# PFLeget/treegp

Measured on AMD Instinct MI355X. Metric: GP solve+predict throughput, 2-D AnisotropicRBF N=65536, higher is better.
Workload: dtype f64

## Files before the change

### treegp_amd/csrc/chol.hip

```cpp
#include "tgp_internal.h"

#include "gemm_tile.h"
#include "potrf128.h"

#ifdef TGP_POTRF_STAMPS
__device__ unsigned long long tgp_gemm_stamps[1024 * 4];
__device__ int tgp_gemm_stamp_grid = 43;
__device__ unsigned long long tgp_queue_stamps[1024 * 4];
__device__ int tgp_queue_stamp_T = 40;
__device__ unsigned long long tgp_mid_stamps[25 * 8];
__device__ int tgp_mid_stamp_base = 5120;
#define TGP_MID_STAMP(i)                                                                                   \
    do {                                                                                                   \
        if (threadIdx.x == 0 && base == tgp_mid_stamp_base && blockIdx.x < 25) tgp_mid_stamps[blockIdx.x * 8 + (i)] = __builtin_amdgcn_s_memrealtime(); \
    } while (0)
#else
#define TGP_MID_STAMP(i) ((void)0)
#endif

namespace {
template <int MODE, int LDB>
__global__ __launch_bounds__(256, 2) void gemm_col_kernel(const double *A, const double *B, double *C) {
    const int64_t t = blockIdx.x;
    TGP_CHAIN_PRIO();
#ifdef TGP_POTRF_STAMPS
    const unsigned long long t_in = __builtin_amdgcn_s_memrealtime();
#endif
    gemm_tile_128<MODE, LDB, TGP_TB>(A + t * 128 * TGP_PW, B, C + t * 128 * TGP_PW);
#ifdef TGP_POTRF_STAMPS
    if (MODE == 0 && threadIdx.x == 0 && (int)gridDim.x == tgp_gemm_stamp_grid) {
        tgp_gemm_stamps[blockIdx.x * 4 + 0] = t_in;
        tgp_gemm_stamps[blockIdx.x * 4 + 1] = __builtin_amdgcn_s_memrealtime();
        tgp_gemm_stamps[blockIdx.x * 4 + 2] = (__builtin_amdgcn_s_getreg(20 | (0 << 6) | (3 << 11)) << 8) | __builtin_amdgcn_s_getreg(4 | (8 << 6) | (7 << 11));
    }
#endif
}

template <int MODE, int LDB>
__global__ __launch_bounds__(256) void gemm_col_small_kernel(const double *A, const double *B, double *C) {
    const int64_t o = (int64_t)blockIdx.x * 16 * TGP_PW;
    TGP_CHAIN_PRIO();
    nt_slice_tile<MODE, TGP_TB, 1>(nt_slice_lds_storage(), A + o, TGP_PW, B, LDB, C + o, TGP_PW, nullptr, nullptr);
}
__device__ __forceinline__ void keep_w_share(double *__restrict__ keep, const double *__restrict__ W0) {
    if (!keep) return;
    constexpr int n2 = TGP_TB * TGP_TB;
    const int per = (n2 + (int)gridDim.x - 1) / (int)gridDim.x;
    const int lo = (int)blockIdx.x * per, hi = lo + per < n2 ? lo + per : n2;
    for (int i = lo + (int)threadIdx.x; i < hi; i += 256)
        reinterpret_cast<double2 *>(keep)[i] = reinterpret_cast<const double2 *>(W0)[i];
}
__global__ __launch_bounds__(256, 2) void panel_tall_kernel(double *rows0, const double *W0, const double *L10, const double *W1,
                                                            double *keep) {
    double *rows = rows0 + (int64_t)blockIdx.x * 128 * TGP_PW;
    TGP_CHAIN_PRIO();
    keep_w_share(keep, W0);
    gemm_tile_128<0, TGP_TB, TGP_TB>(rows, W0, rows);
    __syncthreads();
    gemm_tile_128<1, TGP_PW, TGP_TB>(rows, L10, rows + TGP_TB);
    __syncthreads();
    gemm_tile_128<0, TGP_TB, TGP_TB>(rows + TGP_TB, W1, rows + TGP_TB);
}

__global__ __launch_bounds__(256) void panel_tall_small_kernel(double *rows0, const double *W0, const double *L10, const double *W1,
                                                               double *keep) {
    double *rows = rows0 + (int64_t)blockIdx.x * 16 * TGP_PW;
    TGP_CHAIN_PRIO();
    keep_w_share(keep, W0);
    double *lds = nt_slice_lds_storage();
    nt_slice_tile<0, TGP_TB, 1>(lds, rows, TGP_PW, W0, TGP_TB, rows, TGP_PW, nullptr, nullptr);
    asm volatile("s_waitcnt vmcnt(0)" ::: "memory");
    __syncthreads();
    nt_slice_tile<1, TGP_TB, 1>(lds, rows, TGP_PW, L10, TGP_PW, rows + TGP_TB, TGP_PW, nullptr, nullptr);
    asm volatile("s_waitcnt vmcnt(0)" ::: "memory");
    __syncthreads();
    nt_slice_tile<0, TGP_TB, 1>(lds, rows + TGP_TB, TGP_PW, W1, TGP_TB, rows + TGP_TB, TGP_PW, nullptr, nullptr);
}

__global__ __launch_bounds__(256, 2) void diag_mid_kernel(double *R1, const double *W0) {
    TGP_CHAIN_PRIO();
    gemm_tile_128<0, TGP_TB, TGP_TB>(R1, W0, R1);
    __syncthreads();
    gemm_tile_128<1, TGP_PW, TGP_TB>(R1, R1, R1 + TGP_TB);
}

constexpr unsigned long long PANEL_SPIN_TICKS = 5000000ull;
constexpr int PANEL_SYNC_WORDS = 16;
__device__ __forceinline__ void panel_publish(unsigned *counter) {
    asm volatile("s_waitcnt vmcnt(0)" ::: "memory");
    __syncthreads();
    if (threadIdx.x == 0) {
        __builtin_amdgcn_fence(__ATOMIC_RELEASE, "agent");
        __hip_atomic_fetch_add(counter, 1u, __ATOMIC_RELAXED, __HIP_MEMORY_SCOPE_AGENT);
    }
}
__device__ __forceinline__ bool panel_wait(unsigned *sync, int which, unsigned target, int *info) {
    __shared__ int s_ok;
    if (threadIdx.x == 0) {
        int ok = 1;
        const unsigned long long t0 = __builtin_amdgcn_s_memrealtime();
        unsigned it = 0;
        while (__hip_atomic_load(sync + which, __ATOMIC_RELAXED, __HIP_MEMORY_SCOPE_AGENT) < target) {
            __builtin_amdgcn_s_sleep(1);
            if ((++it & 63u) == 0u) {
                const bool late = __builtin_amdgcn_s_memrealtime() - t0 > PANEL_SPIN_TICKS;
                if (late || __hip_atomic_load(sync + 2, __ATOMIC_RELAXED, __HIP_MEMORY_SCOPE_AGENT) != 0u) {
                    __hip_atomic_store(sync + 2, 1u, __ATOMIC_RELAXED, __HIP_MEMORY_SCOPE_AGENT);
                    if (late) __hip_atomic_store(info, -7, __ATOMIC_RELAXED, __HIP_MEMORY_SCOPE_AGENT);
                    ok = 0;
                    break;
                }
            }
        }
        __builtin_amdgcn_fence(__ATOMIC_ACQUIRE, "agent");
        s_ok = ok;
    }
    __syncthreads();
    const bool ok = s_ok != 0;
    __syncthreads();
    return ok;
}
template <bool SMALLROWS>
__global__ __launch_bounds__(256) void panel_mid_kernel(double *Pk, const double *W0, double *W1, int *info, int base, unsigned *sync) {
    __shared__ __attribute__((aligned(16))) double T[potrf_v2::POTRF_LDS_DOUBLES];
    static_assert(potrf_v2::POTRF_LDS_DOUBLES >= 2 * 2 * 128 * TileDefault::LS, "the GEMM tile's staging fits in potrf128's image");
    static_assert(potrf_v2::POTRF_LDS_DOUBLES >= NT_SLICE_LDS_DOUBLES, "... and the latency tile's");
    TGP_CHAIN_PRIO();
    const int b = blockIdx.x;
    double *R1 = Pk + (int64_t)TGP_TB * TGP_PW;
    TGP_MID_STAMP(0);
    if (b < 8) {
        double *rows = R1 + (int64_t)b * 16 * TGP_PW;
        nt_slice_tile<0, TGP_TB, 1>(T, rows, TGP_PW, W0, TGP_TB, rows, TGP_PW, nullptr, nullptr);
        TGP_MID_STAMP(1);
        panel_publish(sync + 0);
        TGP_MID_STAMP(2);
        return;
    }
    if (b < 24) {
        if (!panel_wait(sync, 0, 8u, info)) return;
        TGP_MID_STAMP(1);
        double *rows = R1 + (int64_t)((b - 8) >> 1) * 16 * TGP_PW;
        const int64_t ch = (int64_t)(b & 1) * 64;
        nt_slice_tile<1, TGP_TB, 1, 64>(T, rows, TGP_PW, R1 + ch * TGP_PW, TGP_PW, rows + TGP_TB + ch, TGP_PW, nullptr, nullptr);
        TGP_MID_STAMP(2);
        panel_publish(sync + 1);
        TGP_MID_STAMP(3);
        return;
    }
    if (b == 24) {
        if (!panel_wait(sync, 1, 16u, info)) return;
        TGP_MID_STAMP(1);
        potrf_v2::potrf128_body<true>(T, R1 + TGP_TB, TGP_PW, W1, info, base + TGP_TB);
        TGP_MID_STAMP(2);
        return;
    }
    if constexpr (SMALLROWS) {
        double *rows = Pk + (int64_t)TGP_PW * TGP_PW + (int64_t)(b - 25) * 16 * TGP_PW;
        nt_slice_tile<0, TGP_TB, 1>(T, rows, TGP_PW, W0, TGP_TB, rows, TGP_PW, nullptr, nullptr);
        asm volatile("s_waitcnt vmcnt(0)" ::: "memory");
        __syncthreads();
        if (!panel_wait(sync, 0, 8u, info)) return;
        nt_slice_tile<1, TGP_TB, 1>(T, rows, TGP_PW, R1, TGP_PW, rows + TGP_TB, TGP_PW, nullptr, nullptr);
    } else {
        double *rows = Pk + (int64_t)TGP_PW * TGP_PW + (int64_t)(b - 25) * 128 * TGP_PW;
        gemm_tile_128_at<0, TGP_TB, TGP_TB>(T, rows, W0, rows);
        __syncthreads();
        if (!panel_wait(sync, 0, 8u, info)) return;
        gemm_tile_128_at<1, TGP_PW, TGP_TB>(T, rows, R1, rows + TGP_TB);
    }
}

template <int NSEG>
__global__ __launch_bounds__(256) void syrk_small_kernel(double *Abase, int64_t Np, int ob, int T, const double *P0,
                                                         const double *P1) {
    const int ri = blockIdx.x;
    const int tj = blockIdx.y;
    if (tj > (ri >> 3) || (ri >> 3) >= T) return;
    TGP_CHAIN_PRIO();
    const int64_t pj = ob + (tj >> 1);
    const int64_t I = (int64_t)TGP_PW * ob + 16 * (int64_t)ri;
    double *C = Abase + panel_off(pj, Np) + (I - pj * TGP_PW) * TGP_PW + (tj & 1) * TGP_TB;
    const int64_t oa = (int64_t)ri * 16 * TGP_PW, obb = (int64_t)tj * TGP_TB * TGP_PW;
    nt_slice_tile<1, TGP_PW, NSEG>(nt_slice_lds_storage(), P0 + oa, TGP_PW, P0 + obb, TGP_PW, C, TGP_PW, NSEG > 1 ? P1 + oa : nullptr,
                                   NSEG > 1 ? P1 + obb : nullptr);
}

template <int NSEG>
__global__ __launch_bounds__(256, 2) void syrk_dtv_kernel(double *Abase, int64_t Np, int ob, int T, int strip, const double *P0,
                                                          const double *P1, int diag_full) {
    int ti, tj;
    if (strip == 0) {
        tilemap(blockIdx.x, T, ti, tj);
        if (ti < 0) return;
    } else {
        tj = (int)(blockIdx.x % strip);
        ti = (int)(blockIdx.x / strip);
        if (ti < tj || ti >= T) return;
    }
// ... 304 lines not shown
        if (n >= slots_per_class) break;
        syrk_distn_tile<NSEG>(((int64_t)n << 3) | xcd, Aloc, loff, kpanel, G, g, S, col_lo, ncol, nrows, M);
        __syncthreads();
    }
}

inline void run_potrf128(hipStream_t st, double *A, int lda, double *W, int *info, int base, bool exclusive = false, bool solo = false) {
    constexpr unsigned image = potrf_v2::POTRF_LDS_BYTES, full = 128 * 1024;
    static const bool attr_ok = [] {
        return hipFuncSetAttribute((const void *)potrf_v2::potrf128_kernel<true>, hipFuncAttributeMaxDynamicSharedMemorySize, (int)full) == hipSuccess &&
               hipFuncSetAttribute((const void *)potrf_v2::potrf128_solo_kernel, hipFuncAttributeMaxDynamicSharedMemorySize, (int)full) == hipSuccess;
    }();
    (void)attr_ok;
    if (exclusive || solo) potrf_v2::potrf128_solo_kernel<<<1, 256, exclusive ? full : image, st>>>(A, lda, W, info, base);
    else potrf_v2::potrf128_kernel<true><<<1, 256, image, st>>>(A, lda, W, info, base);
}
}

namespace {
__global__ void set_identity128_kernel(double *__restrict__ W) {
    const int t = blockIdx.x * 256 + threadIdx.x;
    W[t] = (t >> 7) == (t & 127) ? 1.0 : 0.0;
}

void factor_panel(hipStream_t st, double *Pk, int64_t mk, double *W0, int *d_info, int base, bool exclusive = false,
                  int64_t n_data = -1, unsigned *mid_sync = nullptr, int cu_budget = 0) {
    double *W1 = W0 + TGP_TB * TGP_TB;
    double *R1 = Pk + (int64_t)TGP_TB * TGP_PW;
    const int r1 = (int)((mk - TGP_TB) / TGP_TB);
    static const int small_rows = [] { const char *e = getenv("TGP_SMALL_ROWS"); return e ? atoi(e) : 80; }();
    const bool solo = cu_budget >= 256 && mid_sync != nullptr;
    run_potrf128(st, Pk, TGP_PW, W0, d_info, base, exclusive, solo);
    if (n_data >= 0 && (int64_t)base + TGP_TB >= n_data && mk == TGP_PW) {
        gemm_col_small_kernel<0, TGP_TB><<<8, 256, 0, st>>>(R1, W0, R1);
        set_identity128_kernel<<<64, 256, 0, st>>>(W1);
        return;
    }
    const int r2 = (int)((mk - TGP_PW) / TGP_TB);
    if (mid_sync) {
        constexpr unsigned pad = 128 * 1024 - potrf_v2::POTRF_LDS_DOUBLES * 8;
        static const bool pad_ok = [] {
            return hipFuncSetAttribute((const void *)panel_mid_kernel<true>, hipFuncAttributeMaxDynamicSharedMemorySize, (int)pad) == hipSuccess &&
                   hipFuncSetAttribute((const void *)panel_mid_kernel<false>, hipFuncAttributeMaxDynamicSharedMemorySize, (int)pad) == hipSuccess;
        }();
        const unsigned dyn = (exclusive && pad_ok) ? pad : 0u;
        if (17 + 8 * r2 <= cu_budget) panel_mid_kernel<true><<<25 + 8 * r2, 256, dyn, st>>>(Pk, W0, W1, d_info, base, mid_sync);
        else panel_mid_kernel<false><<<25 + r2, 256, dyn, st>>>(Pk, W0, W1, d_info, base, mid_sync);
    } else if (cu_budget > 0) {
        double *R2 = Pk + (int64_t)TGP_PW * TGP_PW;
        const bool small = 17 + 8 * r2 <= cu_budget;
        gemm_col_small_kernel<0, TGP_TB><<<8, 256, 0, st>>>(R1, W0, R1);
        if (r2 > 0) {
            if (small) gemm_col_small_kernel<0, TGP_TB><<<r2 * 8, 256, 0, st>>>(R2, W0, R2);
            else gemm_col_kernel<0, TGP_TB><<<r2, 256, 0, st>>>(R2, W0, R2);
        }
        gemm_col_small_kernel<1, TGP_PW><<<8, 256, 0, st>>>(R1, R1, R1 + TGP_TB);
        if (r2 > 0) {
            if (small) gemm_col_small_kernel<1, TGP_PW><<<r2 * 8, 256, 0, st>>>(R2, R1, R2 + TGP_TB);
            else gemm_col_kernel<1, TGP_PW><<<r2, 256, 0, st>>>(R2, R1, R2 + TGP_TB);
        }
        run_potrf128(st, R1 + TGP_TB, TGP_PW, W1, d_info, base + TGP_TB, exclusive, solo);
    } else {
        if (r1 <= small_rows) {
            gemm_col_small_kernel<0, TGP_TB><<<r1 * 8, 256, 0, st>>>(R1, W0, R1);
            gemm_col_small_kernel<1, TGP_PW><<<r1 * 8, 256, 0, st>>>(R1, R1, R1 + TGP_TB);
        } else {
            gemm_col_kernel<0, TGP_TB><<<r1, 256, 0, st>>>(R1, W0, R1);
            gemm_col_kernel<1, TGP_PW><<<r1, 256, 0, st>>>(R1, R1, R1 + TGP_TB);
        }
        run_potrf128(st, R1 + TGP_TB, TGP_PW, W1, d_info, base + TGP_TB, exclusive, solo);
    }
    if (r2 > 0) {
        double *R2 = Pk + (int64_t)TGP_PW * TGP_PW + TGP_TB;
        if (r2 <= small_rows) gemm_col_small_kernel<0, TGP_TB><<<r2 * 8, 256, 0, st>>>(R2, W1, R2);
        else gemm_col_kernel<0, TGP_TB><<<r2, 256, 0, st>>>(R2, W1, R2);
    }
}

inline int diag_full() {
    static const int v = [] { const char *e = getenv("TGP_DIAG_FULL"); return e ? (atoi(e) != 0 ? 1 : 0) : 0; }();
    return v;
}

inline int small_t() {
    static const int v = [] { const char *e = getenv("TGP_SMALL_T"); return e ? atoi(e) : 8; }();
    return v;
}

template <int NSEG>
void launch_syrk(hipStream_t st, double *d_A, int64_t Np, int ob, int T, int strip, const double *P0, const double *P1) {
    if (T <= 0) return;
    static const int strip_small_t = [] { const char *e = getenv("TGP_STRIP_SMALL_T"); return e ? atoi(e) : 16; }();
    if (T <= small_t() || (strip > 0 && T <= strip_small_t)) {
        const int cols = strip == 0 ? T : (strip < T ? strip : T);
        syrk_small_kernel<NSEG><<<dim3((unsigned)(T * 8), (unsigned)cols), 256, 0, st>>>(d_A, Np, ob, T, P0, P1);
        return;
    }
    static const int strip64_t = [] { const char *e = getenv("TGP_STRIP64_T"); return e ? atoi(e) : 128; }();
    static const int strip32_t = [] { const char *e = getenv("TGP_STRIP32_T"); return e ? atoi(e) : 64; }();
    if (strip > 0 && T <= strip32_t) {
        syrk_strip32_kernel<NSEG><<<(unsigned)((int64_t)4 * T * strip), 256, 0, st>>>(d_A, Np, ob, T, strip, P0, P1);
        return;
    }
    if (strip > 0 && T <= strip64_t) {
        syrk_strip64_kernel<NSEG><<<(unsigned)((int64_t)2 * T * strip), 256, 0, st>>>(d_A, Np, ob, T, strip, P0, P1);
        return;
    }
    const unsigned gs = strip == 0 ? (unsigned)tilemap_grid(T) : (unsigned)((int64_t)T * strip);
// ... 228 lines not shown
    }
    TGP_HIP(hipGetLastError());
    TGP_HIP(hipMemcpyAsync(ctx->h_info, ctx->d_info, sizeof(int), hipMemcpyDeviceToHost, st));
    ctx->timings[6] = nlaunch;
    ctx->timings[7] = flops;
    ctx->timings[5] = 0.0;
    if (defer_info && !prof) return 0;
    TGP_HIP(hipStreamSynchronize(st));
    if (prof) {
        double tot = 0.0;
        for (int i = 0; i < nlaunch; ++i) {
            float ms = 0.f;
            TGP_HIP(hipEventElapsedTime(&ms, ctx->prof_events[2 * i], ctx->prof_events[2 * i + 1]));
            tot += ms;
        }
        ctx->timings[5] = tot;
    }
    return tgp_potrf_info_rc(ctx, *ctx->h_info);
}

int tgp_potrf_info_rc(tgp_ctx *ctx, int info) {
    if (info >= 0) return info;
    ctx->err = "Cholesky: an in-kernel hand-off timed out (panel_mid_kernel waited 50 ms for workgroups of its own launch); "
               "the factor is incomplete -- TGP_PANEL_MID=0 selects the schedule without in-kernel waits";
    return TGP_RC_HANDOFF;
}

int launch_factor_diag256(tgp_ctx *ctx, double *blk, double *W0, double *W1, int base, bool latency) {
    hipStream_t st = ctx->stream;
    double *R1 = blk + (int64_t)TGP_TB * TGP_PW;
    const bool excl = ctx->chain_exclusive != 0;
    run_potrf128(st, blk, TGP_PW, W0, ctx->d_info, base, excl);
    if (latency) {
        gemm_col_small_kernel<0, TGP_TB><<<8, 256, 0, st>>>(R1, W0, R1);
        gemm_col_small_kernel<1, TGP_PW><<<8, 256, 0, st>>>(R1, R1, R1 + TGP_TB);
    } else {
        diag_mid_kernel<<<1, 256, 0, st>>>(R1, W0);
    }
    run_potrf128(st, R1 + TGP_TB, TGP_PW, W1, ctx->d_info, base + TGP_TB, excl);
    TGP_HIP(hipGetLastError());
    return 0;
}

int launch_trsm_rows(tgp_ctx *ctx, double *rows, int ntiles, const double *Lkk, const double *W0, const double *W1, double *keepW) {
    if (ntiles <= 0) {
        if (keepW) TGP_HIP(hipMemcpyAsync(keepW, W0, (size_t)2 * TGP_TB * TGP_TB * 8, hipMemcpyDeviceToDevice, ctx->stream));
        return 0;
    }
    constexpr int small_max = 24;
    if (ntiles <= small_max)
        panel_tall_small_kernel<<<ntiles * 8, 256, 0, ctx->stream>>>(rows, W0, Lkk + (int64_t)TGP_TB * TGP_PW, W1, keepW);
    else
        panel_tall_kernel<<<ntiles, 256, 0, ctx->stream>>>(rows, W0, Lkk + (int64_t)TGP_TB * TGP_PW, W1, keepW);
    TGP_HIP(hipGetLastError());
    return 0;
}

template <int NSEG>
static void launch_distn(hipStream_t st, unsigned grid, double *d_Aloc, const int64_t *d_loff, int kpanel, int G, int g,
                         const double *const *P, const int *cmax, int col_lo, int ncol, int nrows, const DistMap &M, int nres,
                         unsigned *queue, const double *const *PB) {
    DistSegs<NSEG> S;
    for (int s = 0; s < NSEG; ++s) {
        S.P[s] = P[s];
        S.PB[s] = PB ? PB[s] : P[s];
        S.cmax[s] = cmax[s];
        S.frg[s] = (int)dist_first_round(kpanel + s + 1, g, G);
// ... 158 lines not shown
```

### treegp_amd/csrc/gemm_tile.h

```cpp
#pragma once
#include "tgp_internal.h"

typedef double d4 __attribute__((ext_vector_type(4)));

constexpr int KB = 16;

template <int LSV, bool PRE>
struct TileCfg {
    static constexpr int LS = LSV;
    static constexpr bool PRELOAD = PRE;
};
using TileDefault = TileCfg<17, true>;

using v2u = __attribute__((ext_vector_type(2))) unsigned;
using v4u = __attribute__((ext_vector_type(4))) unsigned;
__device__ __forceinline__ __amdgpu_buffer_rsrc_t tile_rsrc(const double *p, int bytes) {
    return __builtin_amdgcn_make_buffer_rsrc(const_cast<double *>(p), 0, bytes, 0x00020000);
}
__device__ __forceinline__ double buf_ld1(__amdgpu_buffer_rsrc_t r, int voff, int soff) {
    return __builtin_bit_cast(double, __builtin_amdgcn_raw_buffer_load_b64(r, voff, soff, 0));
}
__device__ __forceinline__ double2 buf_ld2(__amdgpu_buffer_rsrc_t r, int voff, int soff) {
    return __builtin_bit_cast(double2, __builtin_amdgcn_raw_buffer_load_b128(r, voff, soff, 0));
}
__device__ __forceinline__ void buf_st1(double x, __amdgpu_buffer_rsrc_t r, int voff, int soff) {
    __builtin_amdgcn_raw_buffer_store_b64(__builtin_bit_cast(v2u, x), r, voff, soff, 0);
}
#ifndef TGP_C_NT
#define TGP_C_NT 1
#endif
__device__ __forceinline__ double buf_ld1_stream(__amdgpu_buffer_rsrc_t r, int voff, int soff) {
    return __builtin_bit_cast(double, __builtin_amdgcn_raw_buffer_load_b64(r, voff, soff, TGP_C_NT ? 2 : 0));
}
__device__ __forceinline__ void buf_st1_stream(double x, __amdgpu_buffer_rsrc_t r, int voff, int soff) {
    __builtin_amdgcn_raw_buffer_store_b64(__builtin_bit_cast(v2u, x), r, voff, soff, TGP_C_NT ? 2 : 0);
}

template <int LS>
__device__ __forceinline__ void lds_put2(double *p, const double2 &v) {
    if constexpr ((LS & 1) == 0) {
        *reinterpret_cast<double2 *>(p) = v;
    } else {
        p[0] = v.x;
        p[1] = v.y;
    }
}

template <int LS>
__device__ __forceinline__ double *tile128_lds_storage() {
    __shared__ __attribute__((aligned(16))) double lds[2 * 2 * 128 * LS];
    return lds;
}

template <int MODE, int LDB, int KDEPTH, typename CFG = TileDefault, int NSEG = 1>
__device__ __forceinline__ void gemm_tile_128_at(double *lds_base, const double *a_ptr, const double *b_ptr, double *c_ptr,
                                                 const double *a1_ptr = nullptr, const double *b1_ptr = nullptr, int nseg_rt = 1,
                                                 int64_t seg_stride_a = 0, int64_t seg_stride_b = 0) {
    constexpr int LDA = TGP_PW, LDC = TGP_PW;
    constexpr int LS = CFG::LS;
    constexpr bool PRELOAD = CFG::PRELOAD && MODE == 1;
    double (*lds)[2][128 * LS] = reinterpret_cast<double (*)[2][128 * LS]>(lds_base);

    const int tid = threadIdx.x;
    const int lane = tid & 63;
    const int w = tid >> 6;
    const int wr = w >> 1, wc = w & 1;
    const int l15 = lane & 15, l4 = lane >> 4;

    const int srow = tid >> 3;
    const int kp = (tid & 7) * 2;
    const __amdgpu_buffer_rsrc_t ra_src = tile_rsrc(a_ptr, 128 * LDA * 8);
    const __amdgpu_buffer_rsrc_t rb_src = tile_rsrc(b_ptr, 128 * LDB * 8);
    const __amdgpu_buffer_rsrc_t ra1_src = tile_rsrc(NSEG > 1 ? a1_ptr : a_ptr, 128 * LDA * 8);
    const __amdgpu_buffer_rsrc_t rb1_src = tile_rsrc(NSEG > 1 ? b1_ptr : b_ptr, 128 * LDB * 8);
    const __amdgpu_buffer_rsrc_t rc_dst = tile_rsrc(c_ptr, 128 * LDC * 8);
    const int va = (srow * LDA + kp) * 8, vb = (srow * LDB + kp) * 8;

    double2 ra[4], rb[4];
#pragma unroll
    for (int s = 0; s < 4; ++s) {
        ra[s] = buf_ld2(ra_src, va, s * 32 * LDA * 8);
        rb[s] = buf_ld2(rb_src, vb, s * 32 * LDB * 8);
    }

    const int vc = ((wr * 64 + l4) * LDC + wc * 64 + l15) * 8;
    d4 acc[4][4];
    if constexpr (PRELOAD) {
#pragma unroll
        for (int m = 0; m < 4; ++m)
#pragma unroll
// ... 63 lines not shown
        if (more) {
#pragma unroll
            for (int s = 0; s < 4; ++s) {
                lds_put2<LS>(&lds[buf ^ 1][0][(srow + 32 * s) * LS + kp], ra[s]);
                lds_put2<LS>(&lds[buf ^ 1][1][(srow + 32 * s) * LS + kp], rb[s]);
            }
        }
        __syncthreads();
    }

#pragma unroll
    for (int m = 0; m < 4; ++m) {
        if constexpr (MODE == 1 && !PRELOAD) {
            double old[4][4];
#pragma unroll
            for (int n = 0; n < 4; ++n)
#pragma unroll
                for (int r = 0; r < 4; ++r) old[n][r] = buf_ld1(rc_dst, vc, ((m * 16 + 4 * r) * LDC + n * 16) * 8);
#pragma unroll
            for (int n = 0; n < 4; ++n)
#pragma unroll
                for (int r = 0; r < 4; ++r)
                    buf_st1(old[n][r] - acc[m][n][r], rc_dst, vc, ((m * 16 + 4 * r) * LDC + n * 16) * 8);
        } else {
#pragma unroll
            for (int n = 0; n < 4; ++n)
#pragma unroll
                for (int r = 0; r < 4; ++r)
                    buf_st1((PRELOAD || MODE == 2) ? -acc[m][n][r] : acc[m][n][r], rc_dst, vc, ((m * 16 + 4 * r) * LDC + n * 16) * 8);
        }
    }
}

template <int MODE, int LDB, int KDEPTH, typename CFG = TileDefault, int NSEG = 1>
__device__ __forceinline__ void gemm_tile_128(const double *a_ptr, const double *b_ptr, double *c_ptr,
                                              const double *a1_ptr = nullptr, const double *b1_ptr = nullptr, int nseg_rt = 1,
                                              int64_t seg_stride_a = 0, int64_t seg_stride_b = 0) {
    gemm_tile_128_at<MODE, LDB, KDEPTH, CFG, NSEG>(tile128_lds_storage<CFG::LS>(), a_ptr, b_ptr, c_ptr, a1_ptr, b1_ptr, nseg_rt,
                                                   seg_stride_a, seg_stride_b);
}


constexpr int DTV_LSB = 18;
__device__ __forceinline__ double *dtv_lds_storage() {
    __shared__ __attribute__((aligned(16))) double lds[2 * 128 * DTV_LSB];
    return lds;
}

template <int NW, int KDEPTH, int NSEG, int MT = 2>
__device__ __forceinline__ void gemm_tile_dtv(const double *a_ptr, const double *b_ptr, double *c_ptr,
                                              const double *a1_ptr, const double *b1_ptr, int nseg_rt = 1,
                                              int64_t seg_stride_a = 0, int64_t seg_stride_b = 0) {
    constexpr int LD = TGP_PW;
    constexpr int LSB = DTV_LSB;
    constexpr int BPT = 16 / NW;
    constexpr int BROWS = 8 * NW;
    double (*ldsB)[128 * LSB] = reinterpret_cast<double (*)[128 * LSB]>(dtv_lds_storage());

    const int tid = threadIdx.x;
    const int lane = tid & 63;
    const int w = __builtin_amdgcn_readfirstlane(tid >> 6);
    const int l15 = lane & 15, l4 = lane >> 4;

    const __amdgpu_buffer_rsrc_t ra0 = tile_rsrc(a_ptr, 16 * MT * NW * LD * 8);
    const __amdgpu_buffer_rsrc_t rb0 = tile_rsrc(b_ptr, 128 * LD * 8);
    const __amdgpu_buffer_rsrc_t ra1 = tile_rsrc(NSEG > 1 ? a1_ptr : a_ptr, 16 * MT * NW * LD * 8);
    const __amdgpu_buffer_rsrc_t rb1 = tile_rsrc(NSEG > 1 ? b1_ptr : b_ptr, 128 * LD * 8);
    const __amdgpu_buffer_rsrc_t rc = tile_rsrc(c_ptr, 16 * MT * NW * LD * 8);
    const int va = ((16 * MT * w + l15) * LD + 2 * l4) * 8;
    const int srow = tid >> 3, kp = (tid & 7) * 2;
    const int vb = (srow * LD + kp) * 8;
    const int vc = ((16 * MT * w + l4) * LD + l15) * 8;
// ... 199 lines not shown
                for (int h = 0; h < 2; ++h) {
                    const int k = (c0 + u) * KB + 8 * h;
                    af[u][h] = *reinterpret_cast<const double2 *>(ap + k);
                    bf[u][0][h] = *reinterpret_cast<const double2 *>(bp + k);
                    bf[u][1][h] = *reinterpret_cast<const double2 *>(bp + (int64_t)16 * ldb + k);
                }
#pragma unroll
            for (int u = 0; u < UN; ++u)
#pragma unroll
                for (int h = 0; h < 2; ++h) {
                    acc[0] = __builtin_amdgcn_mfma_f64_16x16x4f64(af[u][h].x, bf[u][0][h].x, acc[0], 0, 0, 0);
                    acc[1] = __builtin_amdgcn_mfma_f64_16x16x4f64(af[u][h].x, bf[u][1][h].x, acc[1], 0, 0, 0);
                    acc[0] = __builtin_amdgcn_mfma_f64_16x16x4f64(af[u][h].y, bf[u][0][h].y, acc[0], 0, 0, 0);
                    acc[1] = __builtin_amdgcn_mfma_f64_16x16x4f64(af[u][h].y, bf[u][1][h].y, acc[1], 0, 0, 0);
                }
        }
    }
    __syncthreads();
#pragma unroll
    for (int n = 0; n < 2; ++n)
#pragma unroll
        for (int r = 0; r < 4; ++r) {
            double *p = c + (int64_t)(l4 + 4 * r) * ldc + 32 * w + 16 * n + l15;
            if constexpr (MODE == 1) *p = *p - acc[n][r];
            else if constexpr (MODE == 2) *p = -acc[n][r];
            else *p = acc[n][r];
        }
}


typedef double d2v __attribute__((ext_vector_type(2)));
constexpr int NT_SLICE_LS = 66;
constexpr int NT_SLICE_LDS_DOUBLES = (128 + 16) * NT_SLICE_LS;
template <int MODE, int KDEPTH, int NSEG, int NCOL = 128>
__device__ __forceinline__ void nt_slice_tile(double *lds, const double *a, int lda, const double *b, int ldb, double *c, int ldc,
                                              const double *a1, const double *b1) {
    constexpr int LS = NT_SLICE_LS, KBLK = 64;
    constexpr int BPS = KDEPTH / KBLK, NB = NSEG * BPS;
    static_assert(KDEPTH % KBLK == 0 && NB >= 1, "whole blocks of 64 k");
    static_assert(NCOL == 128 || NCOL == 64, "slices of 128 or 64 columns");
    constexpr int NRB = NCOL / 8, NT = NCOL / 64, WC = NCOL / 4;
    const int t = threadIdx.x, lane = t & 63, w = t >> 6;
    const int l15 = lane & 15, l4 = lane >> 4;
    const int prow = t >> 5, pc = 2 * (t & 31);
    d4 acc[2] = {{0.0, 0.0, 0.0, 0.0}, {0.0, 0.0, 0.0, 0.0}};
    d2v rb0[NRB], ra0[2], rb1[NRB], ra1[2];
#define NT_SLICE_FETCH(RB, RA, BLK)                                                                                    \
    {                                                                                                                  \
        constexpr int seg_ = (BLK) / BPS, k0_ = ((BLK) - seg_ * BPS) * KBLK;                                           \
        const double *bp_ = (seg_ ? b1 : b) + k0_ + pc, *ap_ = (seg_ ? a1 : a) + k0_ + pc;                             \
        _Pragma("unroll") for (int i = 0; i < NRB; ++i) RB[i] = *reinterpret_cast<const d2v *>(bp_ + (int64_t)(prow + 8 * i) * ldb); \
        _Pragma("unroll") for (int i = 0; i < 2; ++i) RA[i] = *reinterpret_cast<const d2v *>(ap_ + (int64_t)(prow + 8 * i) * lda);  \
    }
#define NT_SLICE_STAGE(RB, RA)                                                                                         \
    {                                                                                                                  \
        _Pragma("unroll") for (int i = 0; i < NRB; ++i) *reinterpret_cast<d2v *>(lds + (prow + 8 * i) * LS + pc) = RB[i];             \
        _Pragma("unroll") for (int i = 0; i < 2; ++i) *reinterpret_cast<d2v *>(lds + (128 + prow + 8 * i) * LS + pc) = RA[i];        \
    }
    auto multiply = [&] {
        const double *As = lds + (128 + l15) * LS + 2 * l4;
        const double *B0 = lds + (WC * w + l15) * LS + 2 * l4, *B1 = B0 + 16 * LS;
#pragma unroll
        for (int u = 0; u < KBLK / KB; ++u)
#pragma unroll
            for (int h = 0; h < 2; ++h) {
                const int k = u * KB + 8 * h;
                const d2v af = *reinterpret_cast<const d2v *>(As + k);
                const d2v b0 = *reinterpret_cast<const d2v *>(B0 + k);
                if constexpr (NT == 2) {
                    const d2v b1v = *reinterpret_cast<const d2v *>(B1 + k);
                    acc[0] = __builtin_amdgcn_mfma_f64_16x16x4f64(af.x, b0.x, acc[0], 0, 0, 0);
                    acc[1] = __builtin_amdgcn_mfma_f64_16x16x4f64(af.x, b1v.x, acc[1], 0, 0, 0);
                    acc[0] = __builtin_amdgcn_mfma_f64_16x16x4f64(af.y, b0.y, acc[0], 0, 0, 0);
                    acc[1] = __builtin_amdgcn_mfma_f64_16x16x4f64(af.y, b1v.y, acc[1], 0, 0, 0);
                } else {
                    acc[0] = __builtin_amdgcn_mfma_f64_16x16x4f64(af.x, b0.x, acc[0], 0, 0, 0);
                    acc[0] = __builtin_amdgcn_mfma_f64_16x16x4f64(af.y, b0.y, acc[0], 0, 0, 0);
                }
            }
    };
#define NT_SLICE_PAIR(J)                                                                                               \
    if constexpr (2 * (J) < NB) {                                                                                      \
        if constexpr ((J) > 0) __syncthreads();                                                                        \
        NT_SLICE_STAGE(rb0, ra0)                                                                                       \
        if constexpr (2 * (J) + 2 < NB) NT_SLICE_FETCH(rb0, ra0, 2 * (J) + 2)                                          \
        __syncthreads();                                                                                               \
        multiply();                                                                                                    \
        if constexpr (2 * (J) + 1 < NB) {                                                                              \
            __syncthreads();                                                                                           \
            NT_SLICE_STAGE(rb1, ra1)                                                                                   \
            if constexpr (2 * (J) + 3 < NB) NT_SLICE_FETCH(rb1, ra1, 2 * (J) + 3)                                      \
            __syncthreads();                                                                                           \
            multiply();                                                                                                \
        }                                                                                                              \
    }
    static_assert(NB <= 8, "K up to 256, one or two operand pairs");
    NT_SLICE_FETCH(rb0, ra0, 0)
    if constexpr (NB > 1) NT_SLICE_FETCH(rb1, ra1, 1)
    NT_SLICE_PAIR(0)
    NT_SLICE_PAIR(1)
    NT_SLICE_PAIR(2)
    NT_SLICE_PAIR(3)
#undef NT_SLICE_PAIR
#undef NT_SLICE_STAGE
#undef NT_SLICE_FETCH
    __syncthreads();
#pragma unroll
    for (int n = 0; n < NT; ++n)
#pragma unroll
        for (int r = 0; r < 4; ++r) {
            double *p = c + (int64_t)(l4 + 4 * r) * ldc + WC * w + 16 * n + l15;
            if constexpr (MODE == 1) *p = *p - acc[n][r];
            else if constexpr (MODE == 2) *p = -acc[n][r];
            else *p = acc[n][r];
        }
}
__device__ __forceinline__ double *nt_slice_lds_storage() {
    __shared__ __attribute__((aligned(16))) double lds[NT_SLICE_LDS_DOUBLES];
    return lds;
}

template <int NSEG>
struct SegPtrs {
    const double *a[NSEG];
    const double *b[NSEG];
};

template <int NW, int KDEPTH, int NSEG, int MT = 2>
__device__ __forceinline__ void gemm_tile_dtv_segs(const SegPtrs<NSEG> &sp, double *c_ptr) {
    static_assert(NSEG >= 1, "compile-time segment list");
    constexpr int LD = TGP_PW;
    constexpr int LSB = DTV_LSB;
    constexpr int BPT = 16 / NW;
    constexpr int BROWS = 8 * NW;
    double (*ldsB)[128 * LSB] = reinterpret_cast<double (*)[128 * LSB]>(dtv_lds_storage());

    const int tid = threadIdx.x;
    const int lane = tid & 63;
    const int w = __builtin_amdgcn_readfirstlane(tid >> 6);
    const int l15 = lane & 15, l4 = lane >> 4;

    __amdgpu_buffer_rsrc_t ra[NSEG], rb[NSEG];
#pragma unroll
    for (int s = 0; s < NSEG; ++s) {
// ... 278 lines not shown
```

Baseline: 245,800.

## Exploit triangular W in panel X = A W^T tiles to skip zero blocks

Adds a TRIB path to the 128-wide GEMM tile and the 16-row slice tile for the MODE 0 products against the 128x128 W block, which is treated as triangular. Only the (column block, k chunk) pairs that can be nonzero are loaded and multiplied. Column blocks are dealt across wave columns (0,3,4,7 and 1,2,5,6) so the work stays balanced, and the skipped B rows are neither fetched nor staged. This cuts MFMA work and B traffic in the panel solves along the Cholesky critical path. The cost is more complex per-wave control flow, and correctness depends on W being exactly triangular with zeros in the skipped region.

```diff
diff --git a/treegp_amd/csrc/chol.hip b/treegp_amd/csrc/chol.hip
--- a/treegp_amd/csrc/chol.hip
+++ b/treegp_amd/csrc/chol.hip
@@ -19,14 +19,14 @@
 #endif
 
 namespace {
-template <int MODE, int LDB>
+template <int MODE, int LDB, bool TRIB = false>
 __global__ __launch_bounds__(256, 2) void gemm_col_kernel(const double *A, const double *B, double *C) {
     const int64_t t = blockIdx.x;
     TGP_CHAIN_PRIO();
 #ifdef TGP_POTRF_STAMPS
     const unsigned long long t_in = __builtin_amdgcn_s_memrealtime();
 #endif
-    gemm_tile_128<MODE, LDB, TGP_TB>(A + t * 128 * TGP_PW, B, C + t * 128 * TGP_PW);
+    gemm_tile_128<MODE, LDB, TGP_TB, TileDefault, 1, TRIB>(A + t * 128 * TGP_PW, B, C + t * 128 * TGP_PW);
 #ifdef TGP_POTRF_STAMPS
     if (MODE == 0 && threadIdx.x == 0 && (int)gridDim.x == tgp_gemm_stamp_grid) {
         tgp_gemm_stamps[blockIdx.x * 4 + 0] = t_in;
@@ -36,11 +36,11 @@
 #endif
 }
 
-template <int MODE, int LDB>
+template <int MODE, int LDB, bool TRIB = false>
 __global__ __launch_bounds__(256) void gemm_col_small_kernel(const double *A, const double *B, double *C) {
     const int64_t o = (int64_t)blockIdx.x * 16 * TGP_PW;
     TGP_CHAIN_PRIO();
-    nt_slice_tile<MODE, TGP_TB, 1>(nt_slice_lds_storage(), A + o, TGP_PW, B, LDB, C + o, TGP_PW, nullptr, nullptr);
+    nt_slice_tile<MODE, TGP_TB, 1, 128, TRIB>(nt_slice_lds_storage(), A + o, TGP_PW, B, LDB, C + o, TGP_PW, nullptr, nullptr);
 }
 __device__ __forceinline__ void keep_w_share(double *__restrict__ keep, const double *__restrict__ W0) {
     if (!keep) return;
@@ -55,11 +55,11 @@
     double *rows = rows0 + (int64_t)blockIdx.x * 128 * TGP_PW;
     TGP_CHAIN_PRIO();
     keep_w_share(keep, W0);
-    gemm_tile_128<0, TGP_TB, TGP_TB>(rows, W0, rows);
+    gemm_tile_128<0, TGP_TB, TGP_TB, TileDefault, 1, true>(rows, W0, rows);
     __syncthreads();
     gemm_tile_128<1, TGP_PW, TGP_TB>(rows, L10, rows + TGP_TB);
     __syncthreads();
-    gemm_tile_128<0, TGP_TB, TGP_TB>(rows + TGP_TB, W1, rows + TGP_TB);
+    gemm_tile_128<0, TGP_TB, TGP_TB, TileDefault, 1, true>(rows + TGP_TB, W1, rows + TGP_TB);
 }
 
 __global__ __launch_bounds__(256) void panel_tall_small_kernel(double *rows0, const double *W0, const double *L10, const double *W1,
@@ -68,18 +68,18 @@
     TGP_CHAIN_PRIO();
     keep_w_share(keep, W0);
     double *lds = nt_slice_lds_storage();
-    nt_slice_tile<0, TGP_TB, 1>(lds, rows, TGP_PW, W0, TGP_TB, rows, TGP_PW, nullptr, nullptr);
+    nt_slice_tile<0, TGP_TB, 1, 128, true>(lds, rows, TGP_PW, W0, TGP_TB, rows, TGP_PW, nullptr, nullptr);
     asm volatile("s_waitcnt vmcnt(0)" ::: "memory");
     __syncthreads();
     nt_slice_tile<1, TGP_TB, 1>(lds, rows, TGP_PW, L10, TGP_PW, rows + TGP_TB, TGP_PW, nullptr, nullptr);
     asm volatile("s_waitcnt vmcnt(0)" ::: "memory");
     __syncthreads();
-    nt_slice_tile<0, TGP_TB, 1>(lds, rows + TGP_TB, TGP_PW, W1, TGP_TB, rows + TGP_TB, TGP_PW, nullptr, nullptr);
+    nt_slice_tile<0, TGP_TB, 1, 128, true>(lds, rows + TGP_TB, TGP_PW, W1, TGP_TB, rows + TGP_TB, TGP_PW, nullptr, nullptr);
 }
 
 __global__ __launch_bounds__(256, 2) void diag_mid_kernel(double *R1, const double *W0) {
     TGP_CHAIN_PRIO();
-    gemm_tile_128<0, TGP_TB, TGP_TB>(R1, W0, R1);
+    gemm_tile_128<0, TGP_TB, TGP_TB, TileDefault, 1, true>(R1, W0, R1);
     __syncthreads();
     gemm_tile_128<1, TGP_PW, TGP_TB>(R1, R1, R1 + TGP_TB);
 }
@@ -131,7 +131,7 @@
     TGP_MID_STAMP(0);
     if (b < 8) {
         double *rows = R1 + (int64_t)b * 16 * TGP_PW;
-        nt_slice_tile<0, TGP_TB, 1>(T, rows, TGP_PW, W0, TGP_TB, rows, TGP_PW, nullptr, nullptr);
+        nt_slice_tile<0, TGP_TB, 1, 128, true>(T, rows, TGP_PW, W0, TGP_TB, rows, TGP_PW, nullptr, nullptr);
         TGP_MID_STAMP(1);
         panel_publish(sync + 0);
         TGP_MID_STAMP(2);
@@ -157,14 +157,14 @@
     }
     if constexpr (SMALLROWS) {
         double *rows = Pk + (int64_t)TGP_PW * TGP_PW + (int64_t)(b - 25) * 16 * TGP_PW;
-        nt_slice_tile<0, TGP_TB, 1>(T, rows, TGP_PW, W0, TGP_TB, rows, TGP_PW, nullptr, nullptr);
+        nt_slice_tile<0, TGP_TB, 1, 128, true>(T, rows, TGP_PW, W0, TGP_TB, rows, TGP_PW, nullptr, nullptr);
         asm volatile("s_waitcnt vmcnt(0)" ::: "memory");
         __syncthreads();
         if (!panel_wait(sync, 0, 8u, info)) return;
         nt_slice_tile<1, TGP_TB, 1>(T, rows, TGP_PW, R1, TGP_PW, rows + TGP_TB, TGP_PW, nullptr, nullptr);
     } else {
         double *rows = Pk + (int64_t)TGP_PW * TGP_PW + (int64_t)(b - 25) * 128 * TGP_PW;
-        gemm_tile_128_at<0, TGP_TB, TGP_TB>(T, rows, W0, rows);
+        gemm_tile_128_at<0, TGP_TB, TGP_TB, TileDefault, 1, true>(T, rows, W0, rows);
         __syncthreads();
         if (!panel_wait(sync, 0, 8u, info)) return;
         gemm_tile_128_at<1, TGP_PW, TGP_TB>(T, rows, R1, rows + TGP_TB);
@@ -535,7 +535,7 @@
     const bool solo = cu_budget >= 256 && mid_sync != nullptr;
     run_potrf128(st, Pk, TGP_PW, W0, d_info, base, exclusive, solo);
     if (n_data >= 0 && (int64_t)base + TGP_TB >= n_data && mk == TGP_PW) {
-        gemm_col_small_kernel<0, TGP_TB><<<8, 256, 0, st>>>(R1, W0, R1);
+        gemm_col_small_kernel<0, TGP_TB, true><<<8, 256, 0, st>>>(R1, W0, R1);
         set_identity128_kernel<<<64, 256, 0, st>>>(W1);
         return;
     }
@@ -552,10 +552,10 @@
     } else if (cu_budget > 0) {
         double *R2 = Pk + (int64_t)TGP_PW * TGP_PW;
         const bool small = 17 + 8 * r2 <= cu_budget;
-        gemm_col_small_kernel<0, TGP_TB><<<8, 256, 0, st>>>(R1, W0, R1);
+        gemm_col_small_kernel<0, TGP_TB, true><<<8, 256, 0, st>>>(R1, W0, R1);
         if (r2 > 0) {
-            if (small) gemm_col_small_kernel<0, TGP_TB><<<r2 * 8, 256, 0, st>>>(R2, W0, R2);
-            else gemm_col_kernel<0, TGP_TB><<<r2, 256, 0, st>>>(R2, W0, R2);
+            if (small) gemm_col_small_kernel<0, TGP_TB, true><<<r2 * 8, 256, 0, st>>>(R2, W0, R2);
+            else gemm_col_kernel<0, TGP_TB, true><<<r2, 256, 0, st>>>(R2, W0, R2);
         }
         gemm_col_small_kernel<1, TGP_PW><<<8, 256, 0, st>>>(R1, R1, R1 + TGP_TB);
         if (r2 > 0) {
@@ -565,18 +565,18 @@
         run_potrf128(st, R1 + TGP_TB, TGP_PW, W1, d_info, base + TGP_TB, exclusive, solo);
     } else {
         if (r1 <= small_rows) {
-            gemm_col_small_kernel<0, TGP_TB><<<r1 * 8, 256, 0, st>>>(R1, W0, R1);
+            gemm_col_small_kernel<0, TGP_TB, true><<<r1 * 8, 256, 0, st>>>(R1, W0, R1);
             gemm_col_small_kernel<1, TGP_PW><<<r1 * 8, 256, 0, st>>>(R1, R1, R1 + TGP_TB);
         } else {
-            gemm_col_kernel<0, TGP_TB><<<r1, 256, 0, st>>>(R1, W0, R1);
+            gemm_col_kernel<0, TGP_TB, true><<<r1, 256, 0, st>>>(R1, W0, R1);
             gemm_col_kernel<1, TGP_PW><<<r1, 256, 0, st>>>(R1, R1, R1 + TGP_TB);
         }
         run_potrf128(st, R1 + TGP_TB, TGP_PW, W1, d_info, base + TGP_TB, exclusive, solo);
     }
     if (r2 > 0) {
         double *R2 = Pk + (int64_t)TGP_PW * TGP_PW + TGP_TB;
-        if (r2 <= small_rows) gemm_col_small_kernel<0, TGP_TB><<<r2 * 8, 256, 0, st>>>(R2, W1, R2);
-        else gemm_col_kernel<0, TGP_TB><<<r2, 256, 0, st>>>(R2, W1, R2);
+        if (r2 <= small_rows) gemm_col_small_kernel<0, TGP_TB, true><<<r2 * 8, 256, 0, st>>>(R2, W1, R2);
+        else gemm_col_kernel<0, TGP_TB, true><<<r2, 256, 0, st>>>(R2, W1, R2);
     }
 }
 
@@ -871,7 +871,7 @@
     const bool excl = ctx->chain_exclusive != 0;
     run_potrf128(st, blk, TGP_PW, W0, ctx->d_info, base, excl);
     if (latency) {
-        gemm_col_small_kernel<0, TGP_TB><<<8, 256, 0, st>>>(R1, W0, R1);
+        gemm_col_small_kernel<0, TGP_TB, true><<<8, 256, 0, st>>>(R1, W0, R1);
         gemm_col_small_kernel<1, TGP_PW><<<8, 256, 0, st>>>(R1, R1, R1 + TGP_TB);
     } else {
         diag_mid_kernel<<<1, 256, 0, st>>>(R1, W0);
diff --git a/treegp_amd/csrc/gemm_tile.h b/treegp_amd/csrc/gemm_tile.h
--- a/treegp_amd/csrc/gemm_tile.h
+++ b/treegp_amd/csrc/gemm_tile.h
@@ -52,10 +52,146 @@
     return lds;
 }
 
-template <int MODE, int LDB, int KDEPTH, typename CFG = TileDefault, int NSEG = 1>
+constexpr int trib_deal_block(int wc, int n) { return wc == 0 ? (n == 0 ? 0 : n == 1 ? 3 : n == 2 ? 4 : 7) : (n == 0 ? 1 : n == 1 ? 2 : n == 2 ? 5 : 6); }
+constexpr int trib_deal_units(int wc) {
+    int u = 0;
+    for (int n = 0; n < 4; ++n) u += trib_deal_block(wc, n) + 1;
+    return u;
+}
+constexpr int trib_deal_chunk_cost() {
+    int cost = 0;
+    for (int c = 0; c < 8; ++c) {
+        int live[2] = {0, 0};
+        for (int wc = 0; wc < 2; ++wc)
+            for (int n = 0; n < 4; ++n) live[wc] += trib_deal_block(wc, n) >= c ? 1 : 0;
+        cost += live[0] > live[1] ? live[0] : live[1];
+    }
+    return cost;
+}
+constexpr unsigned trib_deal_cover() {
+    unsigned mask = 0;
+    for (int wc = 0; wc < 2; ++wc)
+        for (int n = 0; n < 4; ++n) {
+            const unsigned bit = 1u << trib_deal_block(wc, n);
+            if (mask & bit) return ~0u;
+            mask |= bit;
+        }
+    return mask;
+}
+static_assert(trib_deal_cover() == 0xffu, "the deal covers the eight column blocks, each once");
+static_assert(trib_deal_units(0) == 18 && trib_deal_units(1) == 18, "both wave columns hold 18 of the full tile's 32 (block, chunk) pairs");
+static_assert(trib_deal_chunk_cost() == 20, "chunk by chunk the deal is as short as a deal can be");
+template <int V>
+struct IntC {
+    static constexpr int value = V;
+};
+
+template <int WC, typename CFG>
+__device__ __forceinline__ void tile128_trib_wave(double *lds_base, const double *a_ptr, const double *b_ptr, double *c_ptr) {
+    constexpr int LDA = TGP_PW, LDB = TGP_TB, LDC = TGP_PW;
+    constexpr int LS = CFG::LS;
+    constexpr int NCH = TGP_TB / KB;
+    static_assert(NCH == 8, "eight chunks of 16 k, eight column blocks of 16");
+    double (*lds)[2][128 * LS] = reinterpret_cast<double (*)[2][128 * LS]>(lds_base);
+
+    const int tid = threadIdx.x;
+    const int lane = tid & 63;
+    const int wr = tid >> 7;
+    const int l15 = lane & 15, l4 = lane >> 4;
+    const int srow = tid >> 3;
+    const int kp = (tid & 7) * 2;
+    const __amdgpu_buffer_rsrc_t ra_src = tile_rsrc(a_ptr, 128 * LDA * 8);
+    const __amdgpu_buffer_rsrc_t rb_src = tile_rsrc(b_ptr, 128 * LDB * 8);
+    const __amdgpu_buffer_rsrc_t rc_dst = tile_rsrc(c_ptr, 128 * LDC * 8);
+    const int va = (srow * LDA + kp) * 8, vb = (srow * LDB + kp) * 8;
+
+    double2 ra[4], rb[4];
+#pragma unroll
+    for (int s = 0; s < 4; ++s) {
+        ra[s] = buf_ld2(ra_src, va, s * 32 * LDA * 8);
+        rb[s] = buf_ld2(rb_src, vb, s * 32 * LDB * 8);
+    }
+    d4 acc[4][4];
+#pragma unroll
+    for (int m = 0; m < 4; ++m)
+#pragma unroll
+        for (int n = 0; n < 4; ++n) acc[m][n] = (d4){0.0, 0.0, 0.0, 0.0};
+#pragma unroll
+    for (int s = 0; s < 4; ++s) {
+        lds_put2<LS>(&lds[0][0][(srow + 32 * s) * LS + kp], ra[s]);
+        lds_put2<LS>(&lds[0][1][(srow + 32 * s) * LS + kp], rb[s]);
+    }
+    __syncthreads();
+
+    const int fa = (wr * 64 + l15) * LS + l4;
+    const int fb = l15 * LS + l4;
+    auto chunk = [&](auto cc) {
+        constexpr int C = decltype(cc)::value;
+        constexpr int buf = C & 1;
+        constexpr bool more = (C + 1 < NCH);
+        constexpr int S0 = (C + 1) / 2;
+        if constexpr (more) {
+#pragma unroll
+            for (int s = 0; s < 4; ++s) {
+                ra[s] = buf_ld2(ra_src, va, (s * 32 * LDA + (C + 1) * KB) * 8);
+                if (s >= S0) rb[s] = buf_ld2(rb_src, vb, (s * 32 * LDB + (C + 1) * KB) * 8);
+            }
+        }
+        const double *As = lds[buf][0];
+        const double *Bs = lds[buf][1];
+#pragma unroll
+        for (int k4 = 0; k4 < KB / 4; ++k4) {
+            double af[4], bf[4] = {0.0, 0.0, 0.0, 0.0};
+#pragma unroll
+            for (int m = 0; m < 4; ++m) af[m] = As[fa + m * 16 * LS + k4 * 4];
+#pragma unroll
+            for (int n = 0; n < 4; ++n)
+                if (trib_deal_block(WC, n) >= C) bf[n] = Bs[fb + trib_deal_block(WC, n) * 16 * LS + k4 * 4];
+#pragma unroll
+            for (int m = 0; m < 4; ++m)
+#pragma unroll
+                for (int n = 0; n < 4; ++n)
+                    if (trib_deal_block(WC, n) >= C) acc[m][n] = __builtin_amdgcn_mfma_f64_16x16x4f64(af[m], bf[n], acc[m][n], 0, 0, 0);
+        }
+        __builtin_amdgcn_sched_barrier(0);
+        if constexpr (more) {
+#pragma unroll
+            for (int s = 0; s < 4; ++s) {
+                lds_put2<LS>(&lds[buf ^ 1][0][(srow + 32 * s) * LS + kp], ra[s]);
+                if (s >= S0) lds_put2<LS>(&lds[buf ^ 1][1][(srow + 32 * s) * LS + kp], rb[s]);
+            }
+        }
+        __syncthreads();
+    };
+    chunk(IntC<0>{});
+    chunk(IntC<1>{});
+    chunk(IntC<2>{});
+    chunk(IntC<3>{});
+    chunk(IntC<4>{});
+    chunk(IntC<5>{});
+    chunk(IntC<6>{});
+    chunk(IntC<7>{});
+
+    const int vc = ((wr * 64 + l4) * LDC + l15) * 8;
+#pragma unroll
+    for (int m = 0; m < 4; ++m)
+#pragma unroll
+        for (int n = 0; n < 4; ++n)
+#pragma unroll
+            for (int r = 0; r < 4; ++r)
+                buf_st1(acc[m][n][r], rc_dst, vc, ((m * 16 + 4 * r) * LDC + trib_deal_block(WC, n) * 16) * 8);
+}
+
+template <int MODE, int LDB, int KDEPTH, typename CFG = TileDefault, int NSEG = 1, bool TRIB = false>
 __device__ __forceinline__ void gemm_tile_128_at(double *lds_base, const double *a_ptr, const double *b_ptr, double *c_ptr,
                                                  const double *a1_ptr = nullptr, const double *b1_ptr = nullptr, int nseg_rt = 1,
                                                  int64_t seg_stride_a = 0, int64_t seg_stride_b = 0) {
+    if constexpr (TRIB) {
+        static_assert(MODE == 0 && LDB == TGP_TB && KDEPTH == TGP_TB && NSEG == 1, "X = A W^T with one 128 x 128 W block");
+        if (__builtin_amdgcn_readfirstlane(((int)threadIdx.x >> 6) & 1) == 0) tile128_trib_wave<0, CFG>(lds_base, a_ptr, b_ptr, c_ptr);
+        else tile128_trib_wave<1, CFG>(lds_base, a_ptr, b_ptr, c_ptr);
+        return;
+    }
     constexpr int LDA = TGP_PW, LDC = TGP_PW;
     constexpr int LS = CFG::LS;
     constexpr bool PRELOAD = CFG::PRELOAD && MODE == 1;
@@ -185,12 +321,12 @@
     }
 }
 
-template <int MODE, int LDB, int KDEPTH, typename CFG = TileDefault, int NSEG = 1>
+template <int MODE, int LDB, int KDEPTH, typename CFG = TileDefault, int NSEG = 1, bool TRIB = false>
 __device__ __forceinline__ void gemm_tile_128(const double *a_ptr, const double *b_ptr, double *c_ptr,
                                               const double *a1_ptr = nullptr, const double *b1_ptr = nullptr, int nseg_rt = 1,
                                               int64_t seg_stride_a = 0, int64_t seg_stride_b = 0) {
-    gemm_tile_128_at<MODE, LDB, KDEPTH, CFG, NSEG>(tile128_lds_storage<CFG::LS>(), a_ptr, b_ptr, c_ptr, a1_ptr, b1_ptr, nseg_rt,
-                                                   seg_stride_a, seg_stride_b);
+    gemm_tile_128_at<MODE, LDB, KDEPTH, CFG, NSEG, TRIB>(tile128_lds_storage<CFG::LS>(), a_ptr, b_ptr, c_ptr, a1_ptr, b1_ptr, nseg_rt,
+                                                         seg_stride_a, seg_stride_b);
 }
 
 
@@ -456,13 +592,14 @@
 typedef double d2v __attribute__((ext_vector_type(2)));
 constexpr int NT_SLICE_LS = 66;
 constexpr int NT_SLICE_LDS_DOUBLES = (128 + 16) * NT_SLICE_LS;
-template <int MODE, int KDEPTH, int NSEG, int NCOL = 128>
+template <int MODE, int KDEPTH, int NSEG, int NCOL = 128, bool TRIB = false>
 __device__ __forceinline__ void nt_slice_tile(double *lds, const double *a, int lda, const double *b, int ldb, double *c, int ldc,
                                               const double *a1, const double *b1) {
     constexpr int LS = NT_SLICE_LS, KBLK = 64;
     constexpr int BPS = KDEPTH / KBLK, NB = NSEG * BPS;
     static_assert(KDEPTH % KBLK == 0 && NB >= 1, "whole blocks of 64 k");
     static_assert(NCOL == 128 || NCOL == 64, "slices of 128 or 64 columns");
+    static_assert(!TRIB || (MODE == 0 && KDEPTH == TGP_TB && NSEG == 1 && NCOL == 128), "X = A W^T with one 128 x 128 W block");
     constexpr int NRB = NCOL / 8, NT = NCOL / 64, WC = NCOL / 4;
     const int t = threadIdx.x, lane = t & 63, w = t >> 6;
     const int l15 = lane & 15, l4 = lane >> 4;
@@ -473,16 +610,43 @@
     {                                                                                                                  \
         constexpr int seg_ = (BLK) / BPS, k0_ = ((BLK) - seg_ * BPS) * KBLK;                                           \
         const double *bp_ = (seg_ ? b1 : b) + k0_ + pc, *ap_ = (seg_ ? a1 : a) + k0_ + pc;                             \
-        _Pragma("unroll") for (int i = 0; i < NRB; ++i) RB[i] = *reinterpret_cast<const d2v *>(bp_ + (int64_t)(prow + 8 * i) * ldb); \
+        _Pragma("unroll") for (int i = TRIB ? k0_ / 8 : 0; i < NRB; ++i) RB[i] = *reinterpret_cast<const d2v *>(bp_ + (int64_t)(prow + 8 * i) * ldb); \
         _Pragma("unroll") for (int i = 0; i < 2; ++i) RA[i] = *reinterpret_cast<const d2v *>(ap_ + (int64_t)(prow + 8 * i) * lda);  \
     }
-#define NT_SLICE_STAGE(RB, RA)                                                                                         \
+#define NT_SLICE_STAGE(RB, RA, BLK)                                                                                    \
     {                                                                                                                  \
-        _Pragma("unroll") for (int i = 0; i < NRB; ++i) *reinterpret_cast<d2v *>(lds + (prow + 8 * i) * LS + pc) = RB[i];             \
+        _Pragma("unroll") for (int i = TRIB ? (BLK) * KBLK / 8 : 0; i < NRB; ++i) *reinterpret_cast<d2v *>(lds + (prow + 8 * i) * LS + pc) = RB[i]; \
         _Pragma("unroll") for (int i = 0; i < 2; ++i) *reinterpret_cast<d2v *>(lds + (128 + prow + 8 * i) * LS + pc) = RA[i];        \
     }
-    auto multiply = [&] {
+    const int ws = __builtin_amdgcn_readfirstlane(w);
+    auto multiply = [&](auto blk) {
         const double *As = lds + (128 + l15) * LS + 2 * l4;
+        if constexpr (TRIB) {
+            const double *B0 = lds + (16 * ws + l15) * LS + 2 * l4, *B1 = lds + (16 * (7 - ws) + l15) * LS + 2 * l4;
+#pragma unroll
+            for (int u = 0; u < KBLK / KB; ++u) {
+                const int g = decltype(blk)::value * (KBLK / KB) + u;
+                if (g > 7 - ws) break;
+                const bool both = g <= ws;
+#pragma unroll
+                for (int h = 0; h < 2; ++h) {
+                    const int k = u * KB + 8 * h;
+                    const d2v af = *reinterpret_cast<const d2v *>(As + k);
+                    const d2v b1v = *reinterpret_cast<const d2v *>(B1 + k);
+                    if (both) {
+                        const d2v b0 = *reinterpret_cast<const d2v *>(B0 + k);
+                        acc[0] = __builtin_amdgcn_mfma_f64_16x16x4f64(af.x, b0.x, acc[0], 0, 0, 0);
+                        acc[1] = __builtin_amdgcn_mfma_f64_16x16x4f64(af.x, b1v.x, acc[1], 0, 0, 0);
+                        acc[0] = __builtin_amdgcn_mfma_f64_16x16x4f64(af.y, b0.y, acc[0], 0, 0, 0);
+                        acc[1] = __builtin_amdgcn_mfma_f64_16x16x4f64(af.y, b1v.y, acc[1], 0, 0, 0);
+                    } else {
+                        acc[1] = __builtin_amdgcn_mfma_f64_16x16x4f64(af.x, b1v.x, acc[1], 0, 0, 0);
+                        acc[1] = __builtin_amdgcn_mfma_f64_16x16x4f64(af.y, b1v.y, acc[1], 0, 0, 0);
+                    }
+                }
+            }
+            return;
+        }
         const double *B0 = lds + (WC * w + l15) * LS + 2 * l4, *B1 = B0 + 16 * LS;
 #pragma unroll
         for (int u = 0; u < KBLK / KB; ++u)
@@ -506,16 +670,16 @@
 #define NT_SLICE_PAIR(J)                                                                                               \
     if constexpr (2 * (J) < NB) {                                                                                      \
         if constexpr ((J) > 0) __syncthreads();                                                                        \
-        NT_SLICE_STAGE(rb0, ra0)                                                                                       \
+        NT_SLICE_STAGE(rb0, ra0, 2 * (J))                                                                              \
         if constexpr (2 * (J) + 2 < NB) NT_SLICE_FETCH(rb0, ra0, 2 * (J) + 2)                                          \
         __syncthreads();                                                                                               \
-        multiply();                                                                                                    \
+        multiply(IntC<2 * (J)>{});                                                                                     \
         if constexpr (2 * (J) + 1 < NB) {                                                                              \
             __syncthreads();                                                                                           \
-            NT_SLICE_STAGE(rb1, ra1)                                                                                   \
+            NT_SLICE_STAGE(rb1, ra1, 2 * (J) + 1)                                                                      \
             if constexpr (2 * (J) + 3 < NB) NT_SLICE_FETCH(rb1, ra1, 2 * (J) + 3)                                      \
             __syncthreads();                                                                                           \
-            multiply();                                                                                                \
+            multiply(IntC<2 * (J) + 1>{});                                                                             \
         }                                                                                                              \
     }
     static_assert(NB <= 8, "K up to 256, one or two operand pairs");
@@ -533,7 +697,7 @@
     for (int n = 0; n < NT; ++n)
 #pragma unroll
         for (int r = 0; r < 4; ++r) {
-            double *p = c + (int64_t)(l4 + 4 * r) * ldc + WC * w + 16 * n + l15;
+            double *p = c + (int64_t)(l4 + 4 * r) * ldc + (TRIB ? 16 * (n == 0 ? w : 7 - w) : WC * w + 16 * n) + l15;
             if constexpr (MODE == 1) *p = *p - acc[n][r];
             else if constexpr (MODE == 2) *p = -acc[n][r];
             else *p = acc[n][r];
```

Result: no change. 246,500, median of 6 (+0.3%).
